# StanfordASL/Pigeon.jl

Hardware: AMD Instinct MI355X
Metric: MPC QP solves/sec (N=30 coupled, X1 model) (higher is better)
Workload: dtype f64; 1 GPU; configs[1]: Batch=4096/GPU coupled MPC, N=30 (N_short=10, N_long=20), X1, randomised x0 along skidpadoval, cold start, HJI inactive, fp64; batch_per_gpu=4096, parallelism=single GPU

## Files before the change

### pigeon.jl_amd/csrc/pg_api.hip

```cpp
#include <hip/hip_runtime.h>
#include <math.h>
#include <cmath>
#include <stddef.h>
#include <stdio.h>
#include <stdlib.h>
#include <string.h>
#include <string>
#include <vector>
#include "pg_kernels.hip"

using namespace pg;

struct IndexArray {
    const char *what, *setter; int* d = nullptr; std::vector<int32_t> host;
    int covered() const { return (int)host.size(); }
    void release() { if (d) (void)hipFree(d); d = nullptr; host.clear(); }
};
template <class Host, class Dev> struct SetLib {
    IndexArray idx; std::vector<Host> sets; Dev* d = nullptr;
    bool on() const { return !sets.empty(); }
    const int* index() const { return sets.size() > 1 ? idx.d : (const int*)nullptr; }
    void release() { if (d) (void)hipFree(d); d = nullptr; sets.clear(); idx.release(); }
};
template <class... P> static void dev_release(P*&... p) { ((p ? (void)hipFree(p) : (void)0, p = nullptr), ...); }
// ... 1 lines not shown
    real* buf = nullptr; int steps = 0;
    void clear() { buf = nullptr; steps = 0; }
    HistSlot take() { const HistSlot s = *this; clear(); return s; }
    real* at(int k, int B, int width) const { return (buf && k < steps) ? buf + (size_t)k * B * width : (real*)nullptr; }
};
struct SeedStreams {
    unsigned long long* d = nullptr; bool dirty = true; std::vector<uint64_t> host; uint64_t seed = 0;
    int sync(pg_handle* h);
};

struct pg_handle {
    pg_config cfg;
    DevCfg dc;
    int B = 0;
    int warm_B = 0;
    hipStream_t stream = nullptr;
    int pipeline = 1;
    bool pipe_fault = false;
    int lin_groups = 0;
    int speed_lanes = 0;
    int debug_timeline = 0;
    int lateral_solver = 0;
    int hji_cell_dims = 3;
    int64_t stat_pipelined = 0, stat_split = 0, stat_single = 0, stat_lat_two = 0;
    int solve_parity = 0;
    bool cnt_cleared = false;
    bool lin_done = false;
    int* d_progress = nullptr;
    int64_t fallback_total = 0; int fallback_seen = 0;
    int fuse = 0;
// ... 127 lines not shown
enum SolveCtl {
    CTL_TODO0 = 0, CTL_TODO1 = 1,
    CTL_HAND_BACK = 2,
    CTL_TIMELINE = 4,
    CTL_WHOLE = 5,
    CTL_WORDS = 8
};
enum { ORDER_CNT_WORDS = 2, NODE_COLD_WORDS = 2, PIPE_WORDS = 8 };
static size_t cap_of(const pg_handle* h) { return (size_t)h->cfg.batch_capacity; }
static int* solve_ctl(const pg_handle* h, int word) { return h->d_todo + cap_of(h) + word; }
static int* order_cnt(const pg_handle* h) { return h->d_order + cap_of(h); }                     static int* order_slow(const pg_handle* h) { return order_cnt(h) + ORDER_CNT_WORDS; }
static int* node_heartbeat(const pg_handle* h) { return h->d_node + cap_of(h); }                 static int* node_counts(const pg_handle* h) { return h->d_node + 2 * cap_of(h); }
static int* node_cold(const pg_handle* h, int parity) { return h->d_node + 6 * cap_of(h) + parity; }
static size_t pipe_words(const pg_handle* h) { return cap_of(h) / NODES_IPB + PIPE_WORDS; }
static int* pipe_fault_word(const pg_handle* h, int nbn) { return h->d_progress + nbn; }         static int* pipe_fallbacks(const pg_handle* h) { return h->d_progress + pipe_words(h) - 1; }
static SolveOut solve_out(const pg_handle* h, const int* order) {
    SolveOut O{}; O.sol_x = h->d_solx; O.sol_sigma = h->d_sigma; O.u_out = h->d_u; O.status = h->d_status; O.iters = h->d_iters; O.active = h->d_active; O.mu = h->d_mu;
    O.solved = h->d_solved; O.polish = h->d_polish; O.lam = h->d_lam; O.order_in = order; O.wfail = h->d_wfail;
    return O;
}
template <bool PROF, bool RING, bool FUSE, bool IPM = true>
static void launch_k_solve(pg_handle* h, hipStream_t st, int n, const SolveOut& O, unsigned long long* prof = nullptr) {
    hipLaunchKernelGGL((k_solve<PROF, RING, FUSE, IPM>), dim3(n), dim3(64), h->solve_lds, st, h->dc, h->B, h->d_qp, h->d_nodes, O, prof, h->d_dt, h->d_Mb);
}
enum { LAT_MEM_ANY = 2 };
template <int MEM, int LPI, int HAND>
static void launch_k_solve_lat(pg_handle* h, dim3 grid, size_t lds, hipStream_t st, const SolveOut& O, unsigned long long* prof) {
    if constexpr (MEM == LAT_MEM_ANY) { if (h->lat_mem) launch_k_solve_lat<1, LPI, HAND>(h, grid, lds, st, O, prof); else launch_k_solve_lat<0, LPI, HAND>(h, grid, lds, st, O, prof); }
    else if (h->dc.walls) hipLaunchKernelGGL((k_solve_lat<1, true, MEM != 0, LPI, HAND>), grid, dim3(64), lds, st, h->dc, h->B, h->d_qp, h->d_nodes, O, prof);
    else hipLaunchKernelGGL((k_solve_lat<1, false, MEM != 0, LPI, HAND>), grid, dim3(64), lds, st, h->dc, h->B, h->d_qp, h->d_nodes, O, prof);
// ... 231 lines not shown
        (void)hipFuncSetAttribute((const void*)k_solve<false, false, false>, hipFuncAttributeMaxDynamicSharedMemorySize, (int)h->solve_lds);
        (void)hipFuncSetAttribute((const void*)k_solve<false, false, false, false>, hipFuncAttributeMaxDynamicSharedMemorySize, (int)h->solve_lds);
        (void)hipFuncSetAttribute((const void*)k_solve<false, false, true>, hipFuncAttributeMaxDynamicSharedMemorySize, (int)h->solve_lds);
        (void)hipFuncSetAttribute((const void*)k_solve<false, true, false>, hipFuncAttributeMaxDynamicSharedMemorySize, (int)h->solve_lds);
#ifdef PG_DIAG
        (void)hipFuncSetAttribute((const void*)k_solve<true, false, false>, hipFuncAttributeMaxDynamicSharedMemorySize, (int)h->solve_lds);
        (void)hipFuncSetAttribute((const void*)k_solve<true, true, false>, hipFuncAttributeMaxDynamicSharedMemorySize, (int)h->solve_lds);
#endif
    }
    h->lat_lds = lat_lds_doubles(N) * sizeof(real);
    if (h->solve_lat && h->lat_lds > 64 * 1024) { g_create_error = "horizon too long for k_solve_lat's LDS staging"; free_all(h); delete h; return PG_ERR_INVALID; }
    *out = h;
    return PG_OK;
}

int pg_destroy(pg_handle* h) { if (!h) return PG_ERR_INVALID; (void)hipSetDevice(h->cfg.device); free_all(h); delete h; return PG_OK; }
int pg_get_config(const pg_handle* h, pg_config* out) { if (!h || !out) return PG_ERR_INVALID; *out = h->cfg; return PG_OK; }
int pg_get_u_normalization(const pg_handle* h, double out[2]) {
    if (!h || !out) return PG_ERR_INVALID;
    const bool dec = h->cfg.formulation == PG_DECOUPLED;
    out[0] = dec ? 1.0 : h->cfg.vehicle.delta_max; out[1] = dec ? 1.0 : fmax(-h->cfg.vehicle.Fx_min, h->cfg.vehicle.Fx_max);
    return PG_OK;
}
int pg_precision_bits(void) { return (int)(8 * sizeof(real)); }
int pg_abi_layout(int32_t* out, int32_t n) {
#define OFF(f) (int32_t)offsetof(pg_config, f)
    const int32_t v[] = {(int32_t)sizeof(pg_config), (int32_t)sizeof(pg_vehicle), (int32_t)sizeof(pg_control_params), OFF(control), OFF(N_short), OFF(dt_short), OFF(use_correction_step),
                         OFF(hji_eps), OFF(batch_capacity), OFF(ipm_max_iter), OFF(formulation), OFF(ipm_tol), OFF(ipm_mu0), OFF(walls), OFF(wall_weight), OFF(polish), OFF(polish_rho),
                         OFF(polish_tol), OFF(polish_ipm_tol), OFF(warm_polish), OFF(cold_guess), (int32_t)offsetof(pg_control_params, N_HJI), (int32_t)offsetof(pg_vehicle, kappa_max)};
#undef OFF
    const int32_t cnt = (int32_t)(sizeof(v) / sizeof(v[0]));
    if (out) for (int32_t i = 0; i < cnt && i < n; i++) out[i] = v[i];
    return cnt;
}
int pg_qp_len(const pg_handle* h) { return h ? h->dc.qp_len : PG_ERR_INVALID; }
int pg_set_stream(pg_handle* h, void* s) {
    if (!h) return PG_ERR_INVALID;
    if ((hipStream_t)s != h->stream) { (void)hipSetDevice(h->cfg.device); HIPCHK(h, hipStreamSynchronize(h->stream)); }
    h->stream = (hipStream_t)s;
    return PG_OK;
}
int pg_set_pipeline(pg_handle* h, int32_t mode) { if (!h || mode < 0 || mode > 1) return PG_ERR_INVALID; h->pipeline = mode; return PG_OK; }
int pg_set_fusion(pg_handle* h, int32_t mode) { if (!h || mode < 0 || mode > 2) return PG_ERR_INVALID; h->fuse = mode; return PG_OK; }
namespace {
struct OptRef { int* i; real* r; int64_t* stat; double lo, hi; bool integer; };
static bool find_option(pg_handle* h, const char* name, OptRef* o) {
    DevCfg& C = h->dc;
    *o = OptRef{nullptr, nullptr, nullptr, 0.0, 0.0, true};
    auto I = [&](int* p, double lo, double hi) { o->i = p; o->lo = lo; o->hi = hi; o->integer = true; return true; };
    auto R = [&](real* p, double lo, double hi) { o->r = p; o->lo = lo; o->hi = hi; o->integer = false; return true; };
    auto S = [&](int64_t* p) { o->stat = p; return true; };
    const std::string n(name);
    if (n == "clip_guess") return I(&C.clip_guess, 0, 1);
// ... 298 lines not shown
    if (h->cfg.formulation == PG_COUPLED && !(u.R_dFx > 0.0)) return "a set of a coupled handle needs R_dFx > 0 (the rate weights make the optimum unique)";
    if (u.N_HJI != h->cfg.control.N_HJI) return "N_HJI of a set differs from the handle's (it decides which rows exist: structure, not tuning)";
    return nullptr;
}
static bool same_control(const pg_control_params& a, const pg_control_params& b) {
    return a.V_min == b.V_min && a.V_max == b.V_max && a.k_V == b.k_V && a.k_s == b.k_s && a.deltadot_max == b.deltadot_max && a.Q_ds == b.Q_ds && a.Q_dpsi == b.Q_dpsi && a.Q_e == b.Q_e &&
           a.W_beta == b.W_beta && a.W_r == b.W_r && a.W_HJI == b.W_HJI && a.R_delta == b.R_delta && a.R_ddelta == b.R_ddelta && a.R_Fx == b.R_Fx && a.R_dFx == b.R_dFx && a.N_HJI == b.N_HJI;
}
static int control_sets_changed(pg_handle* h, int n, const pg_control_params* single, const int32_t* index) {
    auto eff = [&](int b) -> const pg_control_params& { return index ? h->cp.sets[(size_t)index[b]] : *single; };
    std::vector<uint8_t> mask((size_t)n, 0); bool any = false;
    for (int b = 0; b < n; b++) if (!same_control(eff(b), h->cp_eff[(size_t)b])) { mask[(size_t)b] = 1; any = true; }
    h->dc.cp_epoch++;
    if (!any) return PG_OK;
    h->warm_B = 0; h->order_B = 0;
    HIPCHK(h, hipMemcpyAsync(h->d_mask, mask.data(), (size_t)n, hipMemcpyHostToDevice, h->stream));
    hipLaunchKernelGGL(k_reset, dim3((n + 255) / 256), dim3(256), 0, h->stream, n, h->d_mask, h->d_solved, h->d_wfail);
    LAUNCH_CHECK(h);
    HIPCHK(h, hipStreamSynchronize(h->stream));
    for (int b = 0; b < n; b++) if (mask[(size_t)b]) h->cp_eff[(size_t)b] = eff(b);
    return PG_OK;
}
int pg_set_control_param_sets(pg_handle* h, int32_t n_sets, const pg_control_params* sets) {
    if (!h) return PG_ERR_INVALID;
    const int rc = setlib_install(h, "pg_set_control_param_sets", h->cp, n_sets, sets, [h](const pg_control_params& u) { return control_set_problem(h, u); },
                                  [h](DevControlRec& r, const pg_control_params& u) { r = make_control_rec(h->cfg.formulation, u); }, n_sets > 1);
    if (rc) return rc;
    DevCfg& C = h->dc; C.n_cp = n_sets; C.cp_sets = h->cp.d; C.cp_idx = nullptr;
    if (n_sets > 1) { C.cp_epoch++; return PG_OK; }
    { const DevControlRec r = make_control_rec(h->cfg.formulation, sets[0]); C.cp = r.cp; C.ux_dummy = r.ux_dummy; }
// ... 385 lines not shown
    HIPCHK(h, hipMalloc((void**)&d, n * sizeof(real)));
    hipLaunchKernelGGL(k_sensor_draws, dim3((unsigned)(((size_t)steps * B + 63) / 64)), dim3(64), 0, h->stream, (int)B, (int)step0, (int)steps, h->sensor.streams.d, (unsigned long long)h->sensor.streams.seed, d);
    std::vector<real> tmp(n);
    hipError_t e = hipGetLastError();
    if (e == hipSuccess) e = hipMemcpyAsync(tmp.data(), d, n * sizeof(real), hipMemcpyDeviceToHost, h->stream);
    if (e == hipSuccess) e = hipStreamSynchronize(h->stream);
    (void)hipFree(d);
    if (e != hipSuccess) { h->err = std::string("pg_sensor_draws: ") + hipGetErrorString(e); return PG_ERR_HIP; }
    for (size_t i = 0; i < n; i++) z[i] = (double)tmp[i];
    return PG_OK;
}
int pg_set_measured_history_dev(pg_handle* h, pg_real_dev* buf, int32_t steps) {
    if (!h) return PG_ERR_INVALID;
    return history_register(h, "pg_set_measured_history_dev", h->sensor.lib, "(the measured state is the true one: record state_hist)", h->sensor.hist, buf, steps);
}
static int check_ready(pg_handle* h);
int pg_get_measured_state(pg_handle* h, double* measured) {
    int rc = check_ready(h); if (rc) return rc;
    if (!h->sensor.valid || !h->sensor.meas) { h->err = "pg_get_measured_state: no rollout step under a sensor library since the inputs were installed"; return PG_ERR_STATE; }
    return down(h, measured, h->sensor.meas, (size_t)h->B * 6);
}

static const char* actuator_field_problem(const pg_actuator_set& s) {
    if (s.delay_steps < 0 || s.delay_steps > PG_ACT_MAX_DELAY) return "delay_steps outside [0, PG_ACT_MAX_DELAY = 16]";
    if (!std::isfinite(s.tau_delta) || s.tau_delta < 0.0) return "tau_delta must be finite and >= 0";
    if (!std::isfinite(s.tau_fx) || s.tau_fx < 0.0) return "tau_fx must be finite and >= 0";
    if (!(s.rate_delta > 0.0)) return "rate_delta must be > 0 or +Inf";
    if (!(s.rate_fx > 0.0)) return "rate_fx must be > 0 or +Inf";
    if (s.feedback != 0 && s.feedback != 1) return "feedback must be 0 or 1";
    return nullptr;
}
// ... 394 lines not shown
        HIPCHK(h, hipMemcpy(rec.data(), d_rec, rec.size() * sizeof(float), hipMemcpyDeviceToHost));
        for (size_t i = 0; i < n; i++) for (int k = 0; k < 7; k++) gradV_out[7 * i + k] = rec[8 * i + 1 + k];
    }
    if (stats) *stats = S;
    if (install) {
        pg_clear_hji_grid(h);
        h->d_hnodes = D.give(d_rec); h->d_knots = D.give(d_kn);
        return hji_install_nodes(h, W);
    }
    return PG_OK;
}

int pg_reset(pg_handle* h, const uint8_t* mask) {
    if (!h) return PG_ERR_INVALID;
    HIPCHK(h, hipSetDevice(h->cfg.device));
    const int cap = h->cfg.batch_capacity;
    h->warm_B = 0; h->order_B = 0;
    if (!mask) { HIPCHK(h, hipMemsetAsync(h->d_solved, 0, (size_t)2 * cap * sizeof(int), h->stream)); return PG_OK; }
    REQUIRE(h, h->B > 0, "pg_reset with a mask needs inputs installed (B known)");
    HIPCHK(h, hipMemcpyAsync(h->d_mask, mask, h->B, hipMemcpyHostToDevice, h->stream));
    hipLaunchKernelGGL(k_reset, dim3((h->B + 255) / 256), dim3(256), 0, h->stream, h->B, h->d_mask, h->d_solved, h->d_wfail);
    LAUNCH_CHECK(h);
    HIPCHK(h, hipStreamSynchronize(h->stream));
    return PG_OK;
}

static void stage_block(pg_handle* h, int32_t B, const double* s_, const double* c_, const double* t0, const double* o_, const double* toff);
static int set_inputs(pg_handle* h, int32_t B, const void* state, const void* control, const double* t0, const void* other, const double* toff, bool host) {
    if (!h) return PG_ERR_INVALID;
    REQUIRE(h, B >= 1 && B <= h->cfg.batch_capacity, "batch size outside [1, batch_capacity]");
    REQUIRE(h, state && control && t0, "state, control and t0 are required");
    HIPCHK(h, hipSetDevice(h->cfg.device));
    h->B = B; h->sim_idx = 0; restart_on_inputs(h);
    const hipMemcpyKind kind = host ? hipMemcpyHostToDevice : hipMemcpyDeviceToDevice;
// ... 17 lines not shown
    HIPCHK(h, hipMemcpyAsync(h->d_control, control, (size_t)B * 3 * sizeof(real), kind, h->stream));
    if (other) HIPCHK(h, hipMemcpyAsync(h->d_other, other, (size_t)B * 4 * sizeof(real), kind, h->stream));
    else HIPCHK(h, hipMemsetAsync(h->d_other, 0, (size_t)B * 4 * sizeof(real), h->stream));
    HIPCHK(h, hipMemcpyAsync(h->d_t0, t0, (size_t)B * 8, kind, h->stream));
    if (toff) HIPCHK(h, hipMemcpyAsync(h->d_toff, toff, (size_t)B * 8, kind, h->stream));
    else HIPCHK(h, hipMemsetAsync(h->d_toff, 0xFF, (size_t)B * 8, h->stream));
    return PG_OK;
}
int pg_set_inputs(pg_handle* h, int32_t B, const double* state, const double* control, const double* t0, const double* other, const double* toff) {
    return set_inputs(h, B, state, control, t0, other, toff, true);
}
int pg_set_inputs_dev(pg_handle* h, int32_t B, const void* state, const void* control, const double* t0, const void* other, const double* toff) {
    return set_inputs(h, B, state, control, t0, other, toff, false);
}

static int check_ready(pg_handle* h) {
    if (!h) return PG_ERR_INVALID;
    if (h->B <= 0) { h->err = "no inputs installed (call pg_set_inputs first)"; return PG_ERR_STATE; }
    if (!h->d_traj) { h->err = "no trajectory installed (call pg_set_trajectory first)"; return PG_ERR_STATE; }
    if (index_covers(h, (size_t)h->dc.n_traj, h->traj_idx) || index_covers(h, (size_t)h->dc.n_cp, h->cp.idx)) return PG_ERR_STATE;
    if (hipSetDevice(h->cfg.device) != hipSuccess) { h->err = "hipSetDevice failed"; return PG_ERR_HIP; }
    return PG_OK;
}

int pg_compute_time_steps(pg_handle* h) {
    int rc = check_ready(h); if (rc) return rc;
    const int B = h->B;
    hipLaunchKernelGGL(k_time_steps, dim3((B + 63) / 64), dim3(64), 0, h->stream, h->dc, B, h->d_t0, h->d_ts, h->d_dt, h->d_prev_ts);
    LAUNCH_CHECK(h);
    return PG_OK;
}
static int launch_nodes(pg_handle* h, bool with_time_grid);
int pg_compute_linearization_nodes(pg_handle* h) {
    int rc = check_ready(h); if (rc) return rc;
    return launch_nodes(h, false);
}
static int launch_hji_rows_compute(pg_handle* h);
// ... 46 lines not shown
#ifdef PG_F32
    if (lpi == 1 && B >= 6144) kern = staged ? k_nodes_linearize<true, 1, 2> : k_nodes_linearize<false, 1, 2>;
#endif
    int nzf = (1024 - nbn + nbt - 1) / nbt;
    if (h->pipe_first > 0) nzf = h->pipe_first;
    if (nzf > h->dc.Ns) nzf = h->dc.Ns;
    if (nzf < 1) nzf = 1;
    unsigned long long pub = 0ull;
    for (int i = 1; i < h->dc.N - 2 && i < 63; i++)
        if (i <= h->dc.Ns ? i % h->pipe_pub_short == 0 : (i - h->dc.Ns) % h->pipe_pub_long == h->pipe_pub_long - 1) pub |= 1ull << i;
    if (h->pipe_fault) pub = 1ull << 63;
    hipLaunchKernelGGL(kern, dim3((unsigned)(nbn + nbt * h->dc.N)), dim3(64), lds, h->stream, h->dc, B, nbn, nzf, pub, h->d_state, h->d_control, h->d_toff, h->d_solved, h->d_sep, h->d_ts,
                       h->d_dt, h->d_prev_ts, h->d_solx, h->d_nodes, F, h->d_naux, h->d_progress, h->d_Mb, h->d_qp, pipe_fault_word(h, nbn), pipe_fallbacks(h));
    LAUNCH_CHECK(h);
    {
        const int* flt = pipe_fault_word(h, nbn);
        hipLaunchKernelGGL(k_nodes_angles, dim3(64), dim3(256), 0, h->stream, h->dc, B, h->d_naux, h->d_nodes, flt);
        const long nz = (long)B * h->dc.Ns * lpi, nr = (long)B * (h->dc.N - h->dc.Ns) * lpi;
        const int nbz = (int)((nz + 63) / 64), nbr = (int)((nr + 63) / 64);
        auto ksplit = lpi == 1 ? k_linearize_split<1> : k_linearize_split<2>;
        hipLaunchKernelGGL(ksplit, dim3(512), dim3(64), 0, h->stream, h->dc, B, nbz, h->d_nodes, h->d_dt, h->d_Mb, h->d_qp, flt, nbz + nbr);
    }
    if (h->dc.n_cp > 1) {
        const long nt = (long)B * h->dc.N;
        hipLaunchKernelGGL(k_rate_limits, dim3((unsigned)((nt + 255) / 256)), dim3(256), 0, h->stream, h->dc, B, h->d_qp);
    }
    h->lin_done = true; h->stat_pipelined++;
    LAUNCH_CHECK(h);
    return PG_OK;
}
static int launch_nodes_cold(pg_handle* h, bool staged, size_t traj_lds, const OrderOut& F) {
    const int B = h->B;
    auto kern = staged ? k_nodes<true> : k_nodes<false>;
    hipLaunchKernelGGL(kern, dim3((B + NODES_IPB - 1) / NODES_IPB), dim3(64), traj_lds, h->stream, h->dc, B, h->d_state, h->d_control, h->d_toff, h->d_solved, h->d_sep, h->d_ts,
                       h->d_dt, h->d_prev_ts, h->d_solx, h->d_nodes, F, h->d_naux);
    LAUNCH_CHECK(h);
    const long nn = (long)B * h->dc.NN;
    hipLaunchKernelGGL(k_nodes_angles, dim3((unsigned)((nn + 255) / 256)), dim3(256), 0, h->stream, h->dc, B, h->d_naux, h->d_nodes);
    LAUNCH_CHECK(h);
    return PG_OK;
}
static int launch_nodes(pg_handle* h, bool with_time_grid) {
    const int B = h->B;
    const bool recheck = h->node_recheck && !h->sg.capturing; h->node_recheck = false;
    const bool pipelined = with_time_grid && pipeline_applies(h);
    h->lin_done = false;
    const bool file = h->dc.formulation != PG_DECOUPLED && h->dc.polish;
    int* const cnt = file ? order_cnt(h) : (int*)nullptr;
    int* const ctl = solve_ctl(h, CTL_TODO0);
    h->cnt_cleared = !h->sg.capturing;
    if (with_time_grid) hipLaunchKernelGGL(k_project<true>, dim3((B * 64 + 255) / 256), dim3(256), 0, h->stream, h->dc, B, h->d_state, h->d_sep, h->d_t0, h->d_ts, h->d_dt, h->d_prev_ts,
                                           pipelined ? h->d_progress : (int*)nullptr, (B + NODES_IPB - 1) / NODES_IPB + 1, cnt, ctl, h->solve_parity);
    else hipLaunchKernelGGL(k_project<false>, dim3((B * 64 + 255) / 256), dim3(256), 0, h->stream, h->dc, B, h->d_state, h->d_sep, (const double*)nullptr, (double*)nullptr, (double*)nullptr,
                            (double*)nullptr, (int*)nullptr, 0, cnt, ctl, h->solve_parity);
    LAUNCH_CHECK(h);
    const bool staged = h->dc.n_traj == 1 && h->traj_L <= 2048;
    const size_t traj_lds = staged ? (size_t)2 * h->traj_L * sizeof(real) : 0;
    const OrderOut F = order_out(h, file ? h->d_order : nullptr);
    h->order_B = file ? B : 0;
    if (h->dc.formulation == PG_DECOUPLED) return launch_nodes_decoupled(h, staged, traj_lds);
    if (h->warm_B >= B) return launch_nodes_warm(h, staged, traj_lds, F, recheck);
    if (pipelined) return launch_nodes_pipelined(h, staged, traj_lds, F);
    return launch_nodes_cold(h, staged, traj_lds, F);
}
static int launch_hji_lookup(pg_handle* h, int B, const real* x7_dev, real* out8_dev) {
    dim3 grid((unsigned)(((size_t)B * 16 + 255) / 256));
    if (h->hv.cdims == 7) hipLaunchKernelGGL(k_hji_lookup<7>, grid, dim3(256), 0, h->stream, h->hv, B, x7_dev, out8_dev);
    else if (h->hv.cdims == 5) hipLaunchKernelGGL(k_hji_lookup<5>, grid, dim3(256), 0, h->stream, h->hv, B, x7_dev, out8_dev);
    else hipLaunchKernelGGL(k_hji_lookup<3>, grid, dim3(256), 0, h->stream, h->hv, B, x7_dev, out8_dev);
// ... 26 lines not shown
    return launch_hji_order(h);
}
#define PG_LIN_PAIR_MAX 1024
static int launch_linearize(pg_handle* h, int n) {
    const int g_env = h->lin_groups;
#ifdef PG_F32
    const int G_small = 2;
#else
    const int G_small = n <= 256 ? 8 : (n <= 512 ? 4 : 2);
#endif
    const int G = (g_env == 1 || g_env == 2 || g_env == 4 || g_env == 8) ? g_env : ((n <= PG_LIN_PAIR_MAX || h->lin_lpi == 2) ? G_small : 1);
    if (G <= 2 && h->dc.Ns > 0 && h->dc.Ns < h->dc.N) {
        const long nz = (long)n * h->dc.Ns * G, nr = (long)n * (h->dc.N - h->dc.Ns) * G;
        const int nbz = (int)((nz + 63) / 64), nbr = (int)((nr + 63) / 64);
        auto ksplit = G == 1 ? k_linearize_split<1> : k_linearize_split<2>;
        hipLaunchKernelGGL(ksplit, dim3((unsigned)(nbz + nbr)), dim3(64), 0, h->stream, h->dc, n, nbz, h->d_nodes, h->d_dt, h->d_Mb, h->d_qp, (const int*)nullptr, 0);
        LAUNCH_CHECK(h);
        return PG_OK;
    }
    const long nl = (long)n * h->dc.N * G;
    const dim3 grid((unsigned)((nl + 63) / 64)), block(64);
    if (G == 1) hipLaunchKernelGGL(k_linearize<8>, grid, block, 0, h->stream, h->dc, n, h->d_nodes, h->d_dt, h->d_Mb, h->d_qp);
    else if (G == 8) hipLaunchKernelGGL(k_linearize<1>, grid, block, 0, h->stream, h->dc, n, h->d_nodes, h->d_dt, h->d_Mb, h->d_qp);
    else if (G == 4) hipLaunchKernelGGL(k_linearize<2>, grid, block, 0, h->stream, h->dc, n, h->d_nodes, h->d_dt, h->d_Mb, h->d_qp);
    else hipLaunchKernelGGL(k_linearize<4>, grid, block, 0, h->stream, h->dc, n, h->d_nodes, h->d_dt, h->d_Mb, h->d_qp);
    LAUNCH_CHECK(h);
    return PG_OK;
}
int pg_update_qp(pg_handle* h) {
    int rc = check_ready(h); if (rc) return rc;
    const int B = h->B; const DevCfg& C = h->dc;
// ... 167 lines not shown
    int rc = check_ready(h); if (rc) return rc;
    if ((rc = launch_hji_policy(h, use_hji_policy))) return rc;
    if (u_out_dev) HIPCHK(h, hipMemcpyAsync(u_out_dev, h->d_pol_u, (size_t)h->B * 3 * sizeof(real), hipMemcpyDeviceToDevice, h->stream));
    if (source_dev) HIPCHK(h, hipMemcpyAsync(source_dev, h->d_pol_src, (size_t)h->B * sizeof(int), hipMemcpyDeviceToDevice, h->stream));
    return PG_OK;
}
int pg_get_next_control_hji(pg_handle* h, int32_t use_hji_policy, double* u_out, int32_t* source, double* u2_policy) {
    int rc = check_ready(h); if (rc) return rc;
    REQUIRE(h, u_out, "u_out is null");
    if ((rc = launch_hji_policy(h, use_hji_policy))) return rc;
    if ((rc = down(h, u_out, h->d_pol_u, (size_t)h->B * 3)) || (rc = down_raw(h, source, h->d_pol_src, (size_t)h->B * sizeof(int))) ||
        (rc = down(h, u2_policy, h->d_pol_u2, (size_t)h->B * 2))) return rc;
    return PG_OK;
}
int pg_step_dev(pg_handle* h, void* u_out_dev) {
    int rc = check_ready(h); if (rc) return rc;
    const bool ev = !h->sg.capturing && h->phase_timing != 0;
    if (ev) HIPCHK(h, hipEventRecord(h->ev[0], h->stream));
    if ((rc = launch_nodes(h, true))) return rc;
    if (ev) HIPCHK(h, hipEventRecord(h->ev[1], h->stream));
    h->u_direct = (real*)u_out_dev; h->u_written = false;
    rc = update_and_solve(h, ev ? h->ev[2] : nullptr);
    h->u_direct = nullptr;
    if (rc) return rc;
    if (!h->u_written && (rc = pg_get_next_control_dev(h, u_out_dev))) return rc;
    if (ev) HIPCHK(h, hipEventRecord(h->ev[3], h->stream));
    h->timing_valid = ev;
    return PG_OK;
}
static int step_compute(pg_handle* h) { const int rc = launch_nodes(h, true); return rc ? rc : update_and_solve(h, nullptr); }
static int check_rollout_args(pg_handle* h, const char* who, int32_t steps, double dt, int32_t human_mode, const void* human_u_dev, bool human_lib) {
// ... 603 lines not shown
```

### pigeon.jl_amd/csrc/pg_kernels.hip

```cpp
#include <hip/hip_runtime.h>
#include <stdint.h>
#include <type_traits>
#include "pg_device.hpp"
#include "pg_julia_range.hpp"

namespace pg {

struct DevCfg {
    DevVehicle veh;
    DevControl cp;
    int Ns, Nl, N, NN;
    tdouble dt_short, dt_long;
    int use_correction_step, nsub;
    int formulation;
    int dbg_poison;
    int dbg_instance;
    real ux_dummy;
    int alias_prev_ts;
    JlRange tg_short, tg_long;
    int time_grid_naive;
    int has_hji;
    real hji_eps;
    real un0, un1;
    real fxmin_n;
// ... 113 lines not shown
    double t0_long = t + C.Ns * C.dt_short;
    if (C.use_correction_step) t0_long = C.dt_long * ceil((t0_long + C.dt_short) / C.dt_long - 1.0);
    auto node_time = [&](int k) __attribute__((always_inline)) -> double {
        if (C.time_grid_naive) return k <= C.Ns ? t + C.dt_short * k : t0_long + C.dt_long * (k - C.Ns);
        return k <= C.Ns ? jl_shifted_elem(C.tg_short, t, k + 1) : jl_shifted_elem(C.tg_long, t0_long, k - C.Ns);
    };
    const double Ti = node_time(i);
    const int n = i + 1;
    const double Tn = node_time(n);
    T[i] = Ti;
    if (i < C.N) D[i] = Tn - Ti;
    if (C.alias_prev_ts) PT[i] = Ti;
}
template <bool TG> __global__ __launch_bounds__(256) void k_project(DevCfg C, int B, const real* __restrict__ state, real* __restrict__ sep, const double* __restrict__ t0, double* __restrict__ ts,
                                                 double* __restrict__ dt, double* __restrict__ prev_ts, int* __restrict__ progress = nullptr, int n_progress = 0, int* __restrict__ order_cnt = nullptr,
                                                 int* __restrict__ solve_ctl = nullptr, int ctl_parity = 0) {
    int wave = (blockIdx.x * blockDim.x + threadIdx.x) >> 6, lane = threadIdx.x & 63;
    if (progress && blockIdx.x == 0) { for (int i = threadIdx.x; i < n_progress; i += blockDim.x) progress[i] = 0; }
    if (order_cnt && blockIdx.x == 0 && threadIdx.x < 2) order_cnt[threadIdx.x] = 0;
    if (solve_ctl && blockIdx.x == 0 && threadIdx.x == 2) solve_ctl[ctl_parity] = 0;
    if (wave >= B) return;
    if constexpr (TG) time_grid_lane(C, lane, t0[wave], ts + (size_t)wave * C.NN, dt + (size_t)wave * C.N, prev_ts + (size_t)wave * C.NN);
    const TrajView T = traj_of(C, wave);
    real x = state[(size_t)wave * 6 + 0], y = state[(size_t)wave * 6 + 1];
    real best = INFINITY; int bi = 0x7fffffff;
    for (int i = lane; i < T.L - 1; i += 64) {
        real d2 = seg_dist2(T.E[i], T.N[i], T.E[i + 1], T.N[i + 1], x, y);
        if (d2 < best) { best = d2; bi = i; }
    }
#pragma unroll
    for (int off = 32; off >= 1; off >>= 1) {
        real ob = __shfl_xor(best, off); int oi = __shfl_xor(bi, off);
// ... 450 lines not shown
                            real* __restrict__ qp) {
    const real* n0 = nodes + ((size_t)b * C.NN + t) * 10;
    linearize_lanes_at<K, ND>(C, b, t, g, live, n0, n0 + 10, dt, hji_Mb, qp);
}
PG_DEV void linearize_pair(const DevCfg& C, int b, int t, int g, bool live, const real* __restrict__ nodes, const tdouble* __restrict__ dt, const real* __restrict__ hji_Mb,
                           real* __restrict__ qp) {
    linearize_lanes<4>(C, b, t, g, live, nodes, dt, hji_Mb, qp);
}
#ifdef PG_F32
#define PG_SPLIT_WAVES 2
#else
#define PG_SPLIT_WAVES 1
#endif
template <int LPI>
__global__ __launch_bounds__(64, PG_SPLIT_WAVES) void k_linearize_split(DevCfg C, int B, int nb_zoh, const real* __restrict__ nodes, const tdouble* __restrict__ dt, const real* __restrict__ hji_Mb,
                                                        real* __restrict__ qp, const int* __restrict__ only_if = nullptr, int nb_total = 0) {
    if (only_if && *only_if == 0) return;
    for (int blk = (int)blockIdx.x; blk < (nb_total ? nb_total : (int)gridDim.x); blk += (int)gridDim.x) {
        const bool zoh = blk < nb_zoh;
        const int nint = zoh ? C.Ns : C.N - C.Ns;
        long gid = (long)(zoh ? blk : blk - nb_zoh) * blockDim.x + threadIdx.x;
        const long per = (long)nint * LPI;
        const bool live = gid < (long)B * per;
        if (!live) gid = (long)B * per - LPI + (gid & (LPI - 1));
        const int b = (int)(gid / per); const int rem = (int)(gid - (long)b * per);
        const int t = (zoh ? 0 : C.Ns) + rem / LPI, g = rem % LPI;
        if (zoh) linearize_lanes<6 / LPI, 6>(C, b, t, g, live, nodes, dt, hji_Mb, qp);
        else linearize_lanes<8 / LPI, 8>(C, b, t, g, live, nodes, dt, hji_Mb, qp);
    }
}
#ifndef PG_LIN_WAVES
#define PG_LIN_WAVES 1
#endif
template <int K>
__global__ __launch_bounds__(64, PG_LIN_WAVES) void k_linearize(DevCfg C, int B, const real* __restrict__ nodes, const tdouble* __restrict__ dt, const real* __restrict__ hji_Mb, real* __restrict__ qp) {
    constexpr int G = 8 / K;
    long gid = (long)blockIdx.x * blockDim.x + threadIdx.x;
    const long per = (long)C.N * G;
    const bool live = gid < (long)B * per;
    if (!live) gid = (long)B * per - G + (gid & (G - 1));
    const int b = (int)(gid / per); const int rem = (int)(gid - (long)b * per);
    linearize_lanes<K>(C, b, rem / G, rem % G, live, nodes, dt, hji_Mb, qp);
}

template <bool STAGED, int LPI, int WAVES = 1> __global__ __launch_bounds__(64, WAVES) void k_nodes_linearize(DevCfg C, int B, int nb_nodes, int nz_first, unsigned long long pub_mask, const real* __restrict__ state, const real* __restrict__ control,
                        const tdouble* __restrict__ toff, const int* __restrict__ solved, const real* __restrict__ sep, const tdouble* __restrict__ ts, const tdouble* __restrict__ dt,
                        const tdouble* __restrict__ prev_ts, const real* __restrict__ prev_x, real* nodes, OrderOut F, real* naux, int* progress, const real* __restrict__ hji_Mb, real* __restrict__ qp, int* fault, int* fault_total) {
    PG_NL_MARK(0, wall_clock64());
    if ((int)blockIdx.x < nb_nodes) {
        nodes_body<STAGED, true>(C, B, (int)blockIdx.x, state, control, toff, solved, sep, ts, dt, prev_ts, prev_x, nodes, F, naux, progress, pub_mask);
        PG_NL_MARK(2, wall_clock64()); PG_NL_MARK(3, 1000ull);
        __threadfence();
        if (threadIdx.x == 0 && !(pub_mask >> 63)) __hip_atomic_store(progress + blockIdx.x, C.NN, __ATOMIC_RELAXED, __HIP_MEMORY_SCOPE_AGENT);
        return;
    }
    extern __shared__ real sh_rec[];
    constexpr int IPB = 64 / LPI;
// ... 20 lines not shown
            __builtin_amdgcn_s_sleep(16);
            if (__hip_atomic_load(fault, __ATOMIC_RELAXED, __HIP_MEMORY_SCOPE_AGENT) != 0 || wall_clock64() > t_give_up) { gave_up = true; break; }
        }
        __builtin_amdgcn_fence(__ATOMIC_ACQUIRE, "agent");
        if (gave_up) {
            if (lane == 0) { __hip_atomic_fetch_add(fault, 1, __ATOMIC_RELAXED, __HIP_MEMORY_SCOPE_AGENT); __hip_atomic_fetch_add(fault_total, 1, __ATOMIC_RELAXED, __HIP_MEMORY_SCOPE_AGENT); }
            return;
        }
    }
    PG_NL_MARK(1, wall_clock64()); PG_NL_MARK(3, (unsigned long long)t);
    const real* n0g = nodes + ((size_t)b * C.NN + t) * 10;
    const real* a0 = naux + ((size_t)b * C.NN + t) * 4;
    real* rec = sh_rec + lane * 20;
#pragma unroll
    for (int k = 0; k < 20; k++) rec[k] = n0g[k];
    {
        const real y0 = a0[0], x0 = a0[1], t0 = a0[2], b0 = a0[3], y1 = a0[4], x1 = a0[5], t1 = a0[6], b1 = a0[7];
        if (y0 == y0) {
            rec[6] = atan2(y0, x0) - atan(t0);
            if (b0 == b0) rec[4] = -atan(b0);
            if (live && g == 0) { real* nd = nodes + ((size_t)b * C.NN + t) * 10; nd[6] = rec[6]; nd[4] = rec[4]; }
        }
        if (y1 == y1) {
            rec[16] = atan2(y1, x1) - atan(t1);
            if (t == C.N - 1) {
                if (b1 == b1) rec[14] = -atan(b1);
                if (live && g == LPI - 1) { real* nd = nodes + ((size_t)b * C.NN + t + 1) * 10; nd[6] = rec[16]; nd[4] = rec[14]; }
            }
        }
    }
    if (t < C.Ns) linearize_lanes_at<6 / LPI, 6, false>(C, b, t, g, live, rec, rec + 10, dt, hji_Mb, qp);
    else linearize_lanes_at<8 / LPI, 8, false>(C, b, t, g, live, rec, rec + 10, dt, hji_Mb, qp);
    PG_NL_MARK(2, wall_clock64());
}

__global__ __launch_bounds__(256) void k_rate_limits(DevCfg C, int B, real* __restrict__ qp) {
    const long gid = (long)blockIdx.x * blockDim.x + threadIdx.x;
    if (gid >= (long)B * C.N) return;
    const int b = (int)(gid / C.N), t = (int)(gid - (long)b * C.N);
    const QpOff o = qp_offsets(C.N);
    real* Q = qp + (size_t)b * C.qp_len;
    const ControlView<false> cv(C, b);
    const real ddot_max = PG_CP(cv, deltadot_max), h_total = Q[o.dt + t];
    Q[o.ddmin + t] = -ddot_max * h_total / C.un0;
    Q[o.ddmax + t] = ddot_max * h_total / C.un0;
}

PG_DEV void advance_ego(const DevCfg& C, real* x, real d, real Fx, real h, int nsub) {
// ... 2078 lines not shown
```

Measured before the change: 7.601 million solves/s.

## Defer unmasked reset into k_project and fuse fallback angle repair with linearize

An unmasked pg_reset no longer issues its own memset. It sets a pending flag, and the zeroing of the solved words is folded into the next k_project launch, with explicit flushes at other entry points and during graph capture. The pipeline fallback path merges the separate k_nodes_angles and k_linearize_split launches into one k_repair_linearize kernel that stages node records in LDS. This removes a memset and a kernel launch per step, at the cost of extra deferred-state bookkeeping and a grid-stride zeroing loop in k_project.

```diff
diff --git a/pigeon.jl_amd/csrc/pg_api.hip b/pigeon.jl_amd/csrc/pg_api.hip
--- a/pigeon.jl_amd/csrc/pg_api.hip
+++ b/pigeon.jl_amd/csrc/pg_api.hip
@@ -39,6 +39,7 @@
     DevCfg dc;
     int B = 0;
     int warm_B = 0;
+    bool reset_pending = false;
     hipStream_t stream = nullptr;
     int pipeline = 1;
     bool pipe_fault = false;
@@ -196,6 +197,12 @@
 static int* node_cold(const pg_handle* h, int parity) { return h->d_node + 6 * cap_of(h) + parity; }
 static size_t pipe_words(const pg_handle* h) { return cap_of(h) / NODES_IPB + PIPE_WORDS; }
 static int* pipe_fault_word(const pg_handle* h, int nbn) { return h->d_progress + nbn; }         static int* pipe_fallbacks(const pg_handle* h) { return h->d_progress + pipe_words(h) - 1; }
+static int flush_reset(pg_handle* h) {
+    if (!h->reset_pending) return PG_OK;
+    HIPCHK(h, hipMemsetAsync(h->d_solved, 0, 2 * cap_of(h) * sizeof(int), h->stream));
+    h->reset_pending = false;
+    return PG_OK;
+}
 static SolveOut solve_out(const pg_handle* h, const int* order) {
     SolveOut O{}; O.sol_x = h->d_solx; O.sol_sigma = h->d_sigma; O.u_out = h->d_u; O.status = h->d_status; O.iters = h->d_iters; O.active = h->d_active; O.mu = h->d_mu;
     O.solved = h->d_solved; O.polish = h->d_polish; O.lam = h->d_lam; O.order_in = order; O.wfail = h->d_wfail;
@@ -457,7 +464,7 @@
     return PG_OK;
 }
 
-int pg_destroy(pg_handle* h) { if (!h) return PG_ERR_INVALID; (void)hipSetDevice(h->cfg.device); free_all(h); delete h; return PG_OK; }
+int pg_destroy(pg_handle* h) { if (!h) return PG_ERR_INVALID; (void)hipSetDevice(h->cfg.device); (void)flush_reset(h); free_all(h); delete h; return PG_OK; }
 int pg_get_config(const pg_handle* h, pg_config* out) { if (!h || !out) return PG_ERR_INVALID; *out = h->cfg; return PG_OK; }
 int pg_get_u_normalization(const pg_handle* h, double out[2]) {
     if (!h || !out) return PG_ERR_INVALID;
@@ -479,7 +486,7 @@
 int pg_qp_len(const pg_handle* h) { return h ? h->dc.qp_len : PG_ERR_INVALID; }
 int pg_set_stream(pg_handle* h, void* s) {
     if (!h) return PG_ERR_INVALID;
-    if ((hipStream_t)s != h->stream) { (void)hipSetDevice(h->cfg.device); HIPCHK(h, hipStreamSynchronize(h->stream)); }
+    if ((hipStream_t)s != h->stream) { (void)hipSetDevice(h->cfg.device); int rc = flush_reset(h); if (rc) return rc; HIPCHK(h, hipStreamSynchronize(h->stream)); }
     h->stream = (hipStream_t)s;
     return PG_OK;
 }
@@ -808,6 +815,7 @@
     h->dc.cp_epoch++;
     if (!any) return PG_OK;
     h->warm_B = 0; h->order_B = 0;
+    { int rc = flush_reset(h); if (rc) return rc; }
     HIPCHK(h, hipMemcpyAsync(h->d_mask, mask.data(), (size_t)n, hipMemcpyHostToDevice, h->stream));
     hipLaunchKernelGGL(k_reset, dim3((n + 255) / 256), dim3(256), 0, h->stream, n, h->d_mask, h->d_solved, h->d_wfail);
     LAUNCH_CHECK(h);
@@ -1223,7 +1231,7 @@
     if (!h) return PG_ERR_INVALID;
     return history_register(h, "pg_set_measured_history_dev", h->sensor.lib, "(the measured state is the true one: record state_hist)", h->sensor.hist, buf, steps);
 }
-static int check_ready(pg_handle* h);
+static int check_ready(pg_handle* h, bool fold_reset = false);
 int pg_get_measured_state(pg_handle* h, double* measured) {
     int rc = check_ready(h); if (rc) return rc;
     if (!h->sensor.valid || !h->sensor.meas) { h->err = "pg_get_measured_state: no rollout step under a sensor library since the inputs were installed"; return PG_ERR_STATE; }
@@ -1648,10 +1656,10 @@
 int pg_reset(pg_handle* h, const uint8_t* mask) {
     if (!h) return PG_ERR_INVALID;
     HIPCHK(h, hipSetDevice(h->cfg.device));
-    const int cap = h->cfg.batch_capacity;
     h->warm_B = 0; h->order_B = 0;
-    if (!mask) { HIPCHK(h, hipMemsetAsync(h->d_solved, 0, (size_t)2 * cap * sizeof(int), h->stream)); return PG_OK; }
+    if (!mask) { h->reset_pending = true; return PG_OK; }
     REQUIRE(h, h->B > 0, "pg_reset with a mask needs inputs installed (B known)");
+    { int rc = flush_reset(h); if (rc) return rc; }
     HIPCHK(h, hipMemcpyAsync(h->d_mask, mask, h->B, hipMemcpyHostToDevice, h->stream));
     hipLaunchKernelGGL(k_reset, dim3((h->B + 255) / 256), dim3(256), 0, h->stream, h->B, h->d_mask, h->d_solved, h->d_wfail);
     LAUNCH_CHECK(h);
@@ -1699,13 +1707,13 @@
     return set_inputs(h, B, state, control, t0, other, toff, false);
 }
 
-static int check_ready(pg_handle* h) {
+static int check_ready(pg_handle* h, bool fold_reset) {
     if (!h) return PG_ERR_INVALID;
     if (h->B <= 0) { h->err = "no inputs installed (call pg_set_inputs first)"; return PG_ERR_STATE; }
     if (!h->d_traj) { h->err = "no trajectory installed (call pg_set_trajectory first)"; return PG_ERR_STATE; }
     if (index_covers(h, (size_t)h->dc.n_traj, h->traj_idx) || index_covers(h, (size_t)h->dc.n_cp, h->cp.idx)) return PG_ERR_STATE;
     if (hipSetDevice(h->cfg.device) != hipSuccess) { h->err = "hipSetDevice failed"; return PG_ERR_HIP; }
-    return PG_OK;
+    return fold_reset ? PG_OK : flush_reset(h);
 }
 
 int pg_compute_time_steps(pg_handle* h) {
@@ -1782,12 +1790,11 @@
                        h->d_dt, h->d_prev_ts, h->d_solx, h->d_nodes, F, h->d_naux, h->d_progress, h->d_Mb, h->d_qp, pipe_fault_word(h, nbn), pipe_fallbacks(h));
     LAUNCH_CHECK(h);
     {
-        const int* flt = pipe_fault_word(h, nbn);
-        hipLaunchKernelGGL(k_nodes_angles, dim3(64), dim3(256), 0, h->stream, h->dc, B, h->d_naux, h->d_nodes, flt);
         const long nz = (long)B * h->dc.Ns * lpi, nr = (long)B * (h->dc.N - h->dc.Ns) * lpi;
         const int nbz = (int)((nz + 63) / 64), nbr = (int)((nr + 63) / 64);
-        auto ksplit = lpi == 1 ? k_linearize_split<1> : k_linearize_split<2>;
-        hipLaunchKernelGGL(ksplit, dim3(512), dim3(64), 0, h->stream, h->dc, B, nbz, h->d_nodes, h->d_dt, h->d_Mb, h->d_qp, flt, nbz + nbr);
+        auto krepair = lpi == 1 ? k_repair_linearize<1> : k_repair_linearize<2>;
+        hipLaunchKernelGGL(krepair, dim3(512), dim3(64), 64 * 20 * sizeof(real), h->stream, h->dc, B, nbz, nbz + nbr, h->d_nodes, h->d_naux, h->d_dt, h->d_Mb, h->d_qp,
+                           (const int*)pipe_fault_word(h, nbn));
     }
     if (h->dc.n_cp > 1) {
         const long nt = (long)B * h->dc.N;
@@ -1817,10 +1824,14 @@
     int* const cnt = file ? order_cnt(h) : (int*)nullptr;
     int* const ctl = solve_ctl(h, CTL_TODO0);
     h->cnt_cleared = !h->sg.capturing;
+    if (h->sg.capturing) { int rc = flush_reset(h); if (rc) return rc; }
+    int* const rst = h->reset_pending ? h->d_solved : (int*)nullptr;
+    const int n_rst = rst ? 2 * (int)cap_of(h) : 0;
+    h->reset_pending = false;
     if (with_time_grid) hipLaunchKernelGGL(k_project<true>, dim3((B * 64 + 255) / 256), dim3(256), 0, h->stream, h->dc, B, h->d_state, h->d_sep, h->d_t0, h->d_ts, h->d_dt, h->d_prev_ts,
-                                           pipelined ? h->d_progress : (int*)nullptr, (B + NODES_IPB - 1) / NODES_IPB + 1, cnt, ctl, h->solve_parity);
+                                           pipelined ? h->d_progress : (int*)nullptr, (B + NODES_IPB - 1) / NODES_IPB + 1, cnt, ctl, h->solve_parity, rst, n_rst);
     else hipLaunchKernelGGL(k_project<false>, dim3((B * 64 + 255) / 256), dim3(256), 0, h->stream, h->dc, B, h->d_state, h->d_sep, (const double*)nullptr, (double*)nullptr, (double*)nullptr,
-                            (double*)nullptr, (int*)nullptr, 0, cnt, ctl, h->solve_parity);
+                            (double*)nullptr, (int*)nullptr, 0, cnt, ctl, h->solve_parity, rst, n_rst);
     LAUNCH_CHECK(h);
     const bool staged = h->dc.n_traj == 1 && h->traj_L <= 2048;
     const size_t traj_lds = staged ? (size_t)2 * h->traj_L * sizeof(real) : 0;
@@ -1877,7 +1888,7 @@
         const long nz = (long)n * h->dc.Ns * G, nr = (long)n * (h->dc.N - h->dc.Ns) * G;
         const int nbz = (int)((nz + 63) / 64), nbr = (int)((nr + 63) / 64);
         auto ksplit = G == 1 ? k_linearize_split<1> : k_linearize_split<2>;
-        hipLaunchKernelGGL(ksplit, dim3((unsigned)(nbz + nbr)), dim3(64), 0, h->stream, h->dc, n, nbz, h->d_nodes, h->d_dt, h->d_Mb, h->d_qp, (const int*)nullptr, 0);
+        hipLaunchKernelGGL(ksplit, dim3((unsigned)(nbz + nbr)), dim3(64), 0, h->stream, h->dc, n, nbz, h->d_nodes, h->d_dt, h->d_Mb, h->d_qp);
         LAUNCH_CHECK(h);
         return PG_OK;
     }
@@ -2075,7 +2086,7 @@
     return PG_OK;
 }
 int pg_step_dev(pg_handle* h, void* u_out_dev) {
-    int rc = check_ready(h); if (rc) return rc;
+    int rc = check_ready(h, true); if (rc) return rc;
     const bool ev = !h->sg.capturing && h->phase_timing != 0;
     if (ev) HIPCHK(h, hipEventRecord(h->ev[0], h->stream));
     if ((rc = launch_nodes(h, true))) return rc;
diff --git a/pigeon.jl_amd/csrc/pg_kernels.hip b/pigeon.jl_amd/csrc/pg_kernels.hip
--- a/pigeon.jl_amd/csrc/pg_kernels.hip
+++ b/pigeon.jl_amd/csrc/pg_kernels.hip
@@ -151,8 +151,9 @@
 }
 template <bool TG> __global__ __launch_bounds__(256) void k_project(DevCfg C, int B, const real* __restrict__ state, real* __restrict__ sep, const double* __restrict__ t0, double* __restrict__ ts,
                                                  double* __restrict__ dt, double* __restrict__ prev_ts, int* __restrict__ progress = nullptr, int n_progress = 0, int* __restrict__ order_cnt = nullptr,
-                                                 int* __restrict__ solve_ctl = nullptr, int ctl_parity = 0) {
+                                                 int* __restrict__ solve_ctl = nullptr, int ctl_parity = 0, int* __restrict__ reset_words = nullptr, int n_reset = 0) {
     int wave = (blockIdx.x * blockDim.x + threadIdx.x) >> 6, lane = threadIdx.x & 63;
+    for (int i = blockIdx.x * blockDim.x + threadIdx.x; i < n_reset; i += gridDim.x * blockDim.x) reset_words[i] = 0;
     if (progress && blockIdx.x == 0) { for (int i = threadIdx.x; i < n_progress; i += blockDim.x) progress[i] = 0; }
     if (order_cnt && blockIdx.x == 0 && threadIdx.x < 2) order_cnt[threadIdx.x] = 0;
     if (solve_ctl && blockIdx.x == 0 && threadIdx.x == 2) solve_ctl[ctl_parity] = 0;
@@ -633,20 +634,18 @@
 #endif
 template <int LPI>
 __global__ __launch_bounds__(64, PG_SPLIT_WAVES) void k_linearize_split(DevCfg C, int B, int nb_zoh, const real* __restrict__ nodes, const tdouble* __restrict__ dt, const real* __restrict__ hji_Mb,
-                                                        real* __restrict__ qp, const int* __restrict__ only_if = nullptr, int nb_total = 0) {
-    if (only_if && *only_if == 0) return;
-    for (int blk = (int)blockIdx.x; blk < (nb_total ? nb_total : (int)gridDim.x); blk += (int)gridDim.x) {
-        const bool zoh = blk < nb_zoh;
-        const int nint = zoh ? C.Ns : C.N - C.Ns;
-        long gid = (long)(zoh ? blk : blk - nb_zoh) * blockDim.x + threadIdx.x;
-        const long per = (long)nint * LPI;
-        const bool live = gid < (long)B * per;
-        if (!live) gid = (long)B * per - LPI + (gid & (LPI - 1));
-        const int b = (int)(gid / per); const int rem = (int)(gid - (long)b * per);
-        const int t = (zoh ? 0 : C.Ns) + rem / LPI, g = rem % LPI;
-        if (zoh) linearize_lanes<6 / LPI, 6>(C, b, t, g, live, nodes, dt, hji_Mb, qp);
-        else linearize_lanes<8 / LPI, 8>(C, b, t, g, live, nodes, dt, hji_Mb, qp);
-    }
+                                                        real* __restrict__ qp) {
+    const int blk = (int)blockIdx.x;
+    const bool zoh = blk < nb_zoh;
+    const int nint = zoh ? C.Ns : C.N - C.Ns;
+    long gid = (long)(zoh ? blk : blk - nb_zoh) * blockDim.x + threadIdx.x;
+    const long per = (long)nint * LPI;
+    const bool live = gid < (long)B * per;
+    if (!live) gid = (long)B * per - LPI + (gid & (LPI - 1));
+    const int b = (int)(gid / per); const int rem = (int)(gid - (long)b * per);
+    const int t = (zoh ? 0 : C.Ns) + rem / LPI, g = rem % LPI;
+    if (zoh) linearize_lanes<6 / LPI, 6>(C, b, t, g, live, nodes, dt, hji_Mb, qp);
+    else linearize_lanes<8 / LPI, 8>(C, b, t, g, live, nodes, dt, hji_Mb, qp);
 }
 #ifndef PG_LIN_WAVES
 #define PG_LIN_WAVES 1
@@ -660,6 +659,22 @@
     if (!live) gid = (long)B * per - G + (gid & (G - 1));
     const int b = (int)(gid / per); const int rem = (int)(gid - (long)b * per);
     linearize_lanes<K>(C, b, rem / G, rem % G, live, nodes, dt, hji_Mb, qp);
+}
+template <int LPI>
+PG_DEV void interval_angles(const DevCfg& C, int b, int t, int g, bool live, const real* a0, real* rec, real* nodes) {
+    const real y0 = a0[0], x0 = a0[1], t0 = a0[2], b0 = a0[3], y1 = a0[4], x1 = a0[5], t1 = a0[6], b1 = a0[7];
+    if (y0 == y0) {
+        rec[6] = atan2(y0, x0) - atan(t0);
+        if (b0 == b0) rec[4] = -atan(b0);
+        if (live && g == 0) { real* nd = nodes + ((size_t)b * C.NN + t) * 10; nd[6] = rec[6]; nd[4] = rec[4]; }
+    }
+    if (y1 == y1) {
+        rec[16] = atan2(y1, x1) - atan(t1);
+        if (t == C.N - 1) {
+            if (b1 == b1) rec[14] = -atan(b1);
+            if (live && g == LPI - 1) { real* nd = nodes + ((size_t)b * C.NN + t + 1) * 10; nd[6] = rec[16]; nd[4] = rec[14]; }
+        }
+    }
 }
 
 template <bool STAGED, int LPI, int WAVES = 1> __global__ __launch_bounds__(64, WAVES) void k_nodes_linearize(DevCfg C, int B, int nb_nodes, int nz_first, unsigned long long pub_mask, const real* __restrict__ state, const real* __restrict__ control,
@@ -710,24 +725,33 @@
     real* rec = sh_rec + lane * 20;
 #pragma unroll
     for (int k = 0; k < 20; k++) rec[k] = n0g[k];
-    {
-        const real y0 = a0[0], x0 = a0[1], t0 = a0[2], b0 = a0[3], y1 = a0[4], x1 = a0[5], t1 = a0[6], b1 = a0[7];
-        if (y0 == y0) {
-            rec[6] = atan2(y0, x0) - atan(t0);
-            if (b0 == b0) rec[4] = -atan(b0);
-            if (live && g == 0) { real* nd = nodes + ((size_t)b * C.NN + t) * 10; nd[6] = rec[6]; nd[4] = rec[4]; }
-        }
-        if (y1 == y1) {
-            rec[16] = atan2(y1, x1) - atan(t1);
-            if (t == C.N - 1) {
-                if (b1 == b1) rec[14] = -atan(b1);
-                if (live && g == LPI - 1) { real* nd = nodes + ((size_t)b * C.NN + t + 1) * 10; nd[6] = rec[16]; nd[4] = rec[14]; }
-            }
-        }
-    }
+    interval_angles<LPI>(C, b, t, g, live, a0, rec, nodes);
     if (t < C.Ns) linearize_lanes_at<6 / LPI, 6, false>(C, b, t, g, live, rec, rec + 10, dt, hji_Mb, qp);
     else linearize_lanes_at<8 / LPI, 8, false>(C, b, t, g, live, rec, rec + 10, dt, hji_Mb, qp);
     PG_NL_MARK(2, wall_clock64());
+}
+template <int LPI>
+__global__ __launch_bounds__(64, PG_SPLIT_WAVES) void k_repair_linearize(DevCfg C, int B, int nb_zoh, int nb_total, real* nodes, const real* __restrict__ naux, const tdouble* __restrict__ dt,
+                                                         const real* __restrict__ hji_Mb, real* __restrict__ qp, const int* __restrict__ only_if) {
+    if (*only_if == 0) return;
+    extern __shared__ real sh_rec[];
+    real* rec = sh_rec + threadIdx.x * 20;
+    for (int blk = (int)blockIdx.x; blk < nb_total; blk += (int)gridDim.x) {
+        const bool zoh = blk < nb_zoh;
+        const int nint = zoh ? C.Ns : C.N - C.Ns;
+        long gid = (long)(zoh ? blk : blk - nb_zoh) * blockDim.x + threadIdx.x;
+        const long per = (long)nint * LPI;
+        const bool live = gid < (long)B * per;
+        if (!live) gid = (long)B * per - LPI + (gid & (LPI - 1));
+        const int b = (int)(gid / per); const int rem = (int)(gid - (long)b * per);
+        const int t = (zoh ? 0 : C.Ns) + rem / LPI, g = rem % LPI;
+        const real* n0g = nodes + ((size_t)b * C.NN + t) * 10;
+#pragma unroll
+        for (int k = 0; k < 20; k++) rec[k] = n0g[k];
+        interval_angles<LPI>(C, b, t, g, live, naux + ((size_t)b * C.NN + t) * 4, rec, nodes);
+        if (zoh) linearize_lanes_at<6 / LPI, 6>(C, b, t, g, live, rec, rec + 10, dt, hji_Mb, qp);
+        else linearize_lanes_at<8 / LPI, 8>(C, b, t, g, live, rec, rec + 10, dt, hji_Mb, qp);
+    }
 }
 
 __global__ __launch_bounds__(256) void k_rate_limits(DevCfg C, int B, real* __restrict__ qp) {
```

Measured after the change: 7.656 million solves/s, median of 6. About the same (+0.7%).
